# edenartlab/sd-lora-trainer

Measured on AMD Instinct MI355X. Metric: training images/sec, SDXL 1024px rank-16 LoRA, 1/2/4/8 GPU (job-parallel), higher is better.
Workload: dtype bf16

## Files before the change

include/sdlt_kernels.h:

```cpp
#ifndef SDLT_KERNELS_H
#define SDLT_KERNELS_H
#include <stdint.h>
#ifdef __cplusplus
extern "C" {
#endif

const char* sdlt_last_error(void);
int sdlt_abi_version(void);
int sdlt_struct_size(int which);

typedef struct sdlt_gemm_batch_item {
  const void* X; const void* W;
  const void* Adown; const void* Bup; void* T_out;
  void* C; void* Ct;
  const float* bias;
  const float* col_scale;
} sdlt_gemm_batch_item;

typedef struct sdlt_gemm_params {
  const void* X; int64_t ldx;
  const void* W; int64_t ldw;
  int32_t M, N, K;
  const void* X2; int64_t ldx2;
  const void* W2; int64_t ldw2;
// ... 16 lines not shown
  void* Ct; int64_t ldct;
  int32_t splitk;
  int32_t ws_cnt_len;
  void* ws_slab; int64_t ws_slab_bytes;
  int32_t stages;
  int32_t accumulate;
  int32_t* ws_cnt;
  int32_t lora_group_n;
  int32_t lora_group_k;
  const sdlt_gemm_batch_item* batch;
  int32_t n_batch;
  int32_t throughput_hint;
  int32_t epi_op; int32_t epi_act;
  void* epi_out; int64_t ld_epi_out;
  const void* epi_in; int64_t ld_epi_in;
  const float* col_scale;
  const float* ln_c1;
  float* ln_stats;
  const float* ln_adapter;
  float ln_eps;
  int32_t ln_nparts;
  const void* ln_parts;
  int32_t x2_group_n;
} sdlt_gemm_params;
int sdlt_gemm_bf16(const sdlt_gemm_params* p, void* stream);


typedef struct sdlt_lora_grad_desc {
  const void* P; int64_t ldp;
  const void* Q; int64_t ldq;
  float* out;
  int32_t M, Cw, R, Rp;
  int32_t rank_major;
  int32_t accumulate;
  int32_t conv, Hin, Win, Cin, Hout, Wout, stride;
  const void* zero;
  int32_t first_block;
  int32_t pad_;
} sdlt_lora_grad_desc;
int sdlt_lora_grad_grouped(const sdlt_lora_grad_desc* descs_dev, const int32_t* block_desc_dev,
                           int32_t n_blocks, int32_t Rp, int32_t mfma, void* stream);
int32_t sdlt_lora_grad_block_cols(void);
int sdlt_lora_grad_wide(const sdlt_lora_grad_desc* descs_dev, const int32_t* block_desc_dev,
                        int32_t n_blocks, int32_t Rp, int32_t mfma, void* stream);

typedef struct sdlt_attn_params {
// ... 417 lines not shown
```

sd-lora-trainer_amd/_lib.py:

```python
import ctypes as C
import os

import torch

_HERE = os.path.dirname(os.path.abspath(__file__))
LIB_PATH = os.environ.get("SDLT_KERNEL_LIB") or os.path.join(_HERE, "libsdlt_kernels.so")

i32, i64, f32, vp = C.c_int32, C.c_int64, C.c_float, C.c_void_p


class GemmParams(C.Structure):
    _fields_ = [
        ("X", vp), ("ldx", i64), ("W", vp), ("ldw", i64),
        ("M", i32), ("N", i32), ("K", i32),
        ("X2", vp), ("ldx2", i64), ("W2", vp), ("ldw2", i64),
        ("K2", i32), ("mode", i32),
        ("Hin", i32), ("Win", i32), ("Cin", i32), ("Hout", i32), ("Wout", i32),
        ("stride", i32), ("ups", i32), ("flip", i32), ("tr", i32),
        ("zero", vp),
        ("Adown", vp), ("ld_adown", i64), ("Bup", vp), ("ld_bup", i64),
        ("T_out", vp), ("ld_t", i64),
        ("lora_R", i32), ("lora_scale", f32), ("alpha", f32),
        ("bias", vp),
        ("rowbias", vp), ("ld_rowbias", i64), ("rows_per_batch", i32),
        ("R", vp), ("ldr", i64),
        ("C", vp), ("ldc", i64),
        ("out_fp32", i32), ("tile", i32),
        ("Ct", vp), ("ldct", i64),
        ("splitk", i32), ("ws_cnt_len", i32), ("ws_slab", vp), ("ws_slab_bytes", i64), ("stages", i32), ("accumulate", i32), ("ws_cnt", vp),
        ("lora_group_n", i32), ("lora_group_k", i32),
        ("batch", vp), ("n_batch", i32), ("throughput_hint", i32),
        ("epi_op", i32), ("epi_act", i32), ("epi_out", vp), ("ld_epi_out", i64), ("epi_in", vp), ("ld_epi_in", i64),
        ("col_scale", vp),
        ("ln_c1", vp), ("ln_stats", vp), ("ln_adapter", vp), ("ln_eps", f32), ("ln_nparts", i32), ("ln_parts", vp),
        ("x2_group_n", i32),
    ]


class LnFoldDesc(C.Structure):
    _fields_ = [("A32", vp), ("lda", i64), ("gamma", vp), ("beta", vp), ("Ag", vp), ("ldag", i64), ("consts", vp), ("rank", i32), ("K", i32)]


class GemmBatchItem(C.Structure):
    _fields_ = [("X", vp), ("W", vp), ("Adown", vp), ("Bup", vp), ("T_out", vp), ("C", vp), ("Ct", vp), ("bias", vp), ("col_scale", vp)]


class SplitsumDesc(C.Structure):
    _fields_ = [("s0", vp), ("s1", vp), ("ld32", i64), ("out0", vp), ("ldo0", i64), ("out1", vp), ("ldo1", i64),
                ("nsplit", i32), ("B", i32), ("Nk", i32), ("Nkp", i32), ("C", i32), ("acc0", i32), ("nblocks", i32), ("pad_", i32)]


class DoraDesc(C.Structure):
    _fields_ = [("W", vp), ("ldw", i64), ("A", vp), ("lda", i64), ("B", vp), ("ldb", i64), ("mag", vp), ("scale", vp), ("Bt", vp), ("ldbt", i64),
                ("B32", vp), ("ldb32", i64), ("N", i32), ("K", i32), ("Rp", i32), ("rank", i32), ("s", f32), ("pad_", i32)]


class DoraWtDesc(C.Structure):
    _fields_ = [("src", vp), ("dst", vp), ("ld", i64), ("scale", vp), ("rows", i32), ("cols", i32), ("period", i32), ("nvalid", i32)]
# ... 264 lines not shown
```

sd-lora-trainer_amd/csrc/gemm.hip:

```cpp
#include <type_traits>
#include "common.h"
#include "../../include/sdlt_kernels.h"

namespace {

constexpr int BK = 64;
constexpr int ROW_BYTES = 128;

struct ConvGeom {
  int Hin, Win, Cin, Hout, Wout, stride, ups, flip, tr;
};

template <int N_>
__device__ __forceinline__ void wait_vmcnt() { asm volatile("s_waitcnt vmcnt(%0)" ::"n"(N_) : "memory"); }

#ifdef SDLT_GEMM_TRACE
__device__ long long g_gemm_tr[16];
#define GTR(i_) do { if (blockIdx.x == 0 && blockIdx.y == 0 && threadIdx.x == 0) g_gemm_tr[i_] = clock64(); } while (0)
#else
#define GTR(i_) do {} while (0)
#endif

template <int MI, int NI, int WN, int MODE, int R16, int NSTAGE, int KG = 0, int BT = 0, int WM = 2, int EPI = 0, int LN = 0>
__global__ __launch_bounds__(64 * WM * WN) void gemm_kernel(const sdlt_gemm_params p) {
  static_assert(!LN || (MODE == 0 && KG == 0 && BT == 0 && R16 <= 1), "folded LayerNorm: plain products, rank pad 16 at most");
  GTR(0);
  const sdlt_gemm_batch_item* bi = BT ? p.batch + blockIdx.y : nullptr;
  const void* pX = (bi && bi->X) ? bi->X : p.X;
  const void* pW = (bi && bi->W) ? bi->W : p.W;
  const void* pAdown = (bi && bi->Adown) ? bi->Adown : p.Adown;
  const void* pBup = (bi && bi->Bup) ? bi->Bup : p.Bup;
  void* pTout = (bi && bi->T_out) ? bi->T_out : p.T_out;
  void* pC = (bi && bi->C) ? bi->C : p.C;
  void* pCt = (bi && bi->Ct) ? bi->Ct : p.Ct;
  const float* pBias = (bi && bi->bias) ? bi->bias : p.bias;
  const float* pCs = R16 ? ((bi && bi->col_scale) ? bi->col_scale : p.col_scale) : nullptr;
  constexpr int NW = WM * WN, NTHR = NW * 64;
  constexpr int BM = WM * MI * 16, BN = WN * NI * 16;
  static_assert(WM == 2 || WM == 4, "wave rows");
  constexpr int XT = BM * ROW_BYTES, WT = BN * ROW_BYTES, AT = (R16 ? R16 * 16 : 0) * ROW_BYTES;
  constexpr int STAGE = XT + WT + AT;
  constexpr int S = NSTAGE;
  constexpr int TW = (KG ? KG * R16 : R16) * 16;
  constexpr int TROW = R16 ? (TW + 4) : 4;
  static_assert(KG == 0 || R16 >= 1, "K-grouped adapters need an adapter");
  extern __shared__ __attribute__((aligned(16))) char smem[];
  char* tsh = smem + (S == 1 ? 2 : S) * STAGE;
  float* lnsh = (float*)(tsh + (R16 ? BM * TROW * 2 : 0));
// ... 244 lines not shown
      lnca = *(const f32x4*)(p.ln_adapter + lgrp * 32 + fk * 4);
      lnab = *(const f32x4*)(p.ln_adapter + lgrp * 32 + 16 + fk * 4);
    }
  }
  f32x4 lnp[LN == 2 ? 8 : 1];
  if constexpr (LN == 2) {
#pragma unroll
    for (int i = 0; i < 8; ++i) {
      const int tr = tid < BM ? tid : 0;
      const int m = m0 + tr < p.M ? m0 + tr : p.M - 1;
      lnp[i] = *(const f32x4*)((const float*)p.ln_parts + ((size_t)m * p.ln_nparts + (2 * i < p.ln_nparts ? 2 * i : 0)) * 2);
    }
  }
  constexpr int CST = BN + 4;
  constexpr int REGION = (S == 1 ? 2 : S) * STAGE;
  constexpr int CROWS = BM * CST * 4 <= REGION ? BM : (BM / 2 * CST * 4 <= REGION ? BM / 2 : BM / 4);
  static_assert(CROWS * CST * 4 <= REGION && CROWS % 16 == 0, "staged epilogue does not fit the staging LDS");
  constexpr int NCH = BN / 8;
  constexpr int QPP = CROWS * NCH / NTHR;
  constexpr int RIT = (BM / CROWS) * QPP;
  constexpr bool RPRE = RIT <= 4 && QPP * NTHR == CROWS * NCH;
  const bool vec_ok = ((p.ldc & 3) == 0) && (p.R == nullptr || (p.ldr & 3) == 0) &&
                      (p.rowbias == nullptr || (p.ld_rowbias & 3) == 0);
  const bool staged = EPI != 0 ||
                      ((long)p.M * p.N >= (1l << 20) && !p.out_fp32 && pCt == nullptr && vec_ok && (p.ldc & 7) == 0 && (p.N & 7) == 0 &&
                       (p.R == nullptr || (p.ldr & 7) == 0) && (((uintptr_t)pC | (uintptr_t)p.R) & 15) == 0);
  uint4 rpre[RPRE ? RIT : 1];
  const bool rpre_on = RPRE && staged && p.R != nullptr && splitk == 1;
  if (rpre_on) {
#pragma unroll
    for (int t = 0; t < RIT; ++t) {
      const int it = tid + (t % QPP) * NTHR, row = it / NCH, ch = it - row * NCH;
      const int m = m0 + (t / QPP) * CROWS + row, n = n0 + ch * 8;
      rpre[t] = *(const uint4*)((const bf16_t*)p.R + (size_t)(m < p.M ? m : p.M - 1) * p.ldr + (n < p.N ? n : 0));
    }
  }

  GTR(14);
  f32x4 acc[NI][MI];
#pragma unroll
  for (int a = 0; a < NI; ++a)
#pragma unroll
    for (int b = 0; b < MI; ++b) acc[a][b] = (f32x4){0.f, 0.f, 0.f, 0.f};
  constexpr int TMI = MI >= WN ? MI / WN : 1;
  const bool t_active = wn * TMI < MI;
  f32x4 tacc[R16 ? R16 : 1][TMI];
#pragma unroll
// ... 408 lines not shown
          o.x = pack2bf(dh[0], dh[1]); o.y = pack2bf(dh[2], dh[3]); o.z = pack2bf(dh[4], dh[5]); o.w = pack2bf(dh[6], dh[7]);
          *(uint4*)dst = o;
          o.x = pack2bf(dgt[0], dgt[1]); o.y = pack2bf(dgt[2], dgt[3]); o.z = pack2bf(dgt[4], dgt[5]); o.w = pack2bf(dgt[6], dgt[7]);
          *(uint4*)(dst + 16) = o;
          continue;
        }
        if constexpr (EPI == 4) {
          const uint4 pv = *(const uint4*)((const bf16_t*)p.epi_in + (size_t)m * p.ld_epi_in + n);
          const uint32_t* pp = (const uint32_t*)&pv;
          float v8[8] = {lo[0], lo[1], lo[2], lo[3], hi[0], hi[1], hi[2], hi[3]};
#pragma unroll
          for (int j = 0; j < 8; ++j) {
            const float x = bf2f((pp[j >> 1] >> ((j & 1) * 16)) & 0xffff);
            float d;
            if (p.epi_act == 1) { const float sg = 1.f / (1.f + __expf(-1.702f * x)); d = sg + 1.702f * x * sg * (1.f - sg); }
            else d = dgelu_f(x);
            v8[j] *= d;
          }
          lo = (f32x4){v8[0], v8[1], v8[2], v8[3]};
          hi = (f32x4){v8[4], v8[5], v8[6], v8[7]};
        }
        o.x = pack2bf(lo[0], lo[1]); o.y = pack2bf(lo[2], lo[3]); o.z = pack2bf(hi[0], hi[1]); o.w = pack2bf(hi[2], hi[3]);
        *(uint4*)((bf16_t*)pC + (size_t)m * p.ldc + n) = o;
        if constexpr (EPI == 3) {
          float v8[8] = {lo[0], lo[1], lo[2], lo[3], hi[0], hi[1], hi[2], hi[3]};
#pragma unroll
          for (int j = 0; j < 8; ++j) v8[j] = p.epi_act == 1 ? v8[j] / (1.f + __expf(-1.702f * v8[j])) : gelu_f(v8[j]);
          uint4 q;
          q.x = pack2bf(v8[0], v8[1]); q.y = pack2bf(v8[2], v8[3]); q.z = pack2bf(v8[4], v8[5]); q.w = pack2bf(v8[6], v8[7]);
          *(uint4*)((bf16_t*)p.epi_out + (size_t)m * p.ld_epi_out + n) = q;
        }
        if (EPI == 1 && ((n >> 4) & 1) == 0) {
          const f32x4 glo = *(const f32x4*)(src + 16), ghi = *(const f32x4*)(src + 20);
          uint4 q;
          q.x = pack2bf(lo[0] * gelu_f(glo[0]), lo[1] * gelu_f(glo[1])); q.y = pack2bf(lo[2] * gelu_f(glo[2]), lo[3] * gelu_f(glo[3]));
          q.z = pack2bf(hi[0] * gelu_f(ghi[0]), hi[1] * gelu_f(ghi[1])); q.w = pack2bf(hi[2] * gelu_f(ghi[2]), hi[3] * gelu_f(ghi[3]));
          *(uint4*)((bf16_t*)p.epi_out + (size_t)m * p.ld_epi_out + (n >> 5) * 16 + (n & 15)) = q;
        }
      }
      if (pass + 1 < BM / CROWS) __syncthreads();
    }
    GTR(11);
    return;
  }
#endif
#pragma unroll
// ... 38 lines not shown
          *(float4*)((float*)pC + (size_t)m * p.ldc + n) = make_float4(v[0], v[1], v[2], v[3]);
        } else {
          uint2 o;
          o.x = pack2bf(v[0], v[1]); o.y = pack2bf(v[2], v[3]);
          *(uint2*)((bf16_t*)pC + (size_t)m * p.ldc + n) = o;
        }
      } else {
#pragma unroll
        for (int r = 0; r < 4; ++r) {
          if (n + r >= p.N) break;
          float x = v[r] + (pBias ? biasf[a][r] : 0.f);
          if (p.rowbias) x += bf2f(((const bf16_t*)p.rowbias)[(size_t)brow * p.ld_rowbias + n + r]);
          if (p.R) x += bf2f(((const bf16_t*)p.R)[(size_t)m * p.ldr + n + r]);
          if (pCt) ((bf16_t*)pCt)[(size_t)(n + r) * p.ldct + m] = f2bf(x);
          if (p.out_fp32) ((float*)pC)[(size_t)m * p.ldc + n + r] = p.accumulate ? ((float*)pC)[(size_t)m * p.ldc + n + r] + x : x;
          else ((bf16_t*)pC)[(size_t)m * p.ldc + n + r] = f2bf(x);
        }
      }
    }
  }
  GTR(11);
}

template <int MI, int NI, int WN, int MODE, int R16, int NSREQ, int KG = 0, int BT = 0, int WM = 2, int EPI = 0, int LN = 0>
int launch(const sdlt_gemm_params& p, hipStream_t stream) {
  constexpr int NTHR = 64 * WM * WN;
  constexpr int BM = WM * MI * 16, BN = WN * NI * 16;
  constexpr int STAGE = (BM + BN + R16 * 16) * ROW_BYTES;
  constexpr int TSH = (R16 ? BM * ((KG ? KG * R16 : R16) * 16 + 4) * 2 : 0) + (LN ? BM * 8 : 0);
  constexpr int NS = NSREQ <= 2 ? NSREQ : ((4 * STAGE + TSH <= 160 * 1024) ? 4 : ((3 * STAGE + TSH <= 160 * 1024) ? 3 : 2));
  constexpr int NBUF = NS == 1 ? 2 : NS;
  if constexpr (NBUF * STAGE + TSH > 160 * 1024) {
    SDLT_FAIL(SDLT_ERR_UNSUPPORTED, "sdlt_gemm_bf16: tile %dx%d with LoRA rank pad %d does not fit the 160 KB LDS", BM, BN, R16 * 16);
  } else {
  const int smem = NBUF * STAGE + TSH;
  if (sdlt_raise_smem((const void*)gemm_kernel<MI, NI, WN, MODE, R16, NS, KG, BT, WM, EPI, LN>, smem))
    SDLT_FAIL(SDLT_ERR_LAUNCH, "sdlt_gemm_bf16: cannot raise the dynamic LDS limit to %d bytes", smem);
  const int nbm = (p.M + BM - 1) / BM, nbn = (p.N + BN - 1) / BN;
  const int splitk = p.splitk > 1 ? p.splitk : 1;
  if (splitk > 1) {
    constexpr int TMI = MI >= WN ? MI / WN : 1;
    const size_t slab_bytes = (size_t)(NI * MI + (R16 ? R16 * TMI : 0)) * NTHR * 16;
    if (!p.ws_slab || !p.ws_cnt || (size_t)nbm * nbn * splitk * slab_bytes > (size_t)p.ws_slab_bytes || nbm * nbn > p.ws_cnt_len)
      SDLT_FAIL(SDLT_ERR_SHAPE, "sdlt_gemm_bf16: split-K workspace too small (%d tiles x %d splits x %zu B)", nbm * nbn, splitk, slab_bytes);
  }
  hipLaunchKernelGGL((gemm_kernel<MI, NI, WN, MODE, R16, NS, KG, BT, WM, EPI, LN>), dim3(nbm * nbn * splitk, BT ? p.n_batch : 1), dim3(NTHR), smem, stream, p);
  }
  return SDLT_OK;
}

void tile_dims(int tile, int& bm, int& bn) {
  switch (tile) {
    case 7: bm = 256; bn = 160; break;
    case 8: bm = 128; bn = 160; break;
    case 1: case 5: bm = 128; bn = 128; break;
    case 2: bm = 64; bn = 128; break;
    case 4: bm = 256; bn = 128; break;
    case 6: bm = 256; bn = 256; break;
    default: bm = 64; bn = 64; break;
  }
}

template <int MODE, int R16>
int dispatch_tile(const sdlt_gemm_params& pin, hipStream_t s) {
  sdlt_gemm_params p = pin;
  if (p.lora_group_k > 0) {
    const int G = p.K / p.lora_group_k;
    const long t128 = (long)((p.M + 127) / 128) * ((p.N + 127) / 128);
    p.splitk = (pin.splitk == G || (pin.splitk == 0 && G > 1 && t128 * G <= 320 && p.ws_slab && p.ws_cnt)) ? G : 1;
  }
  if (p.batch) p.splitk = 1;
  if (p.ln_c1) p.splitk = 1;
  const int ktot = p.K + p.K2;
  if (p.tile == 0) {
    const long t128 = (long)((p.M + 127) / 128) * ((p.N + 127) / 128);
    const int nk = ktot / BK;
    const bool ws = p.ws_slab && p.ws_cnt;
    if (R16 <= 1 && !p.batch && !p.lora_group_k && p.N % 160 == 0 && p.M > 128 && !p.throughput_hint) {
      const long t7 = (long)((p.M + 255) / 256) * (p.N / 160), t8 = (long)((p.M + 127) / 128) * (p.N / 160);
      if (MODE == 0 && R16 == 0 && ktot <= 2560) {
        if (t7 >= 256) p.tile = 7;
        else if (t8 >= 224) p.tile = 8;
      } else if (MODE == 0 && R16 == 1 && !p.lora_group_n && ktot <= 640 && t8 >= 224 && t8 <= 320) {
        p.tile = 8;
      } else if (MODE != 0 && (t8 == 256 || t8 == 128 || t8 == 64)) {
        const int sk = (int)(256 / t8);
        if (sk == 1 || (ws && !p.splitk && nk / sk >= 16)) { p.tile = 8; if (sk > 1) p.splitk = sk; }
      }
      if (p.tile && !p.splitk) p.splitk = 1;
    }
    if (p.tile) {}
    else if (p.M <= 64) p.tile = p.N > 64 ? 2 : 3;
    else if (p.N <= 64) p.tile = 3;
    else if (p.M <= 128) {
      p.tile = 3;
// ... 48 lines not shown
    const long tiles = (long)((p.M + bm - 1) / bm) * ((p.N + bn - 1) / bn);
    const int nk = ktot / BK;
    int sk = 1;
    if (p.ws_slab && p.ws_cnt && tiles <= 96) {
      sk = (int)((256 + tiles / 2) / tiles);
      const int min_steps = tiles <= 32 ? 3 : 8;
      if (sk > nk / min_steps) sk = nk / min_steps;
      if (sk > 16) sk = 16;
      if (sk < 1) sk = 1;
    }
    p.splitk = sk;
  }
#define SDLT_TILE_CASES(NSV)                                         \
  switch (p.tile) {                                                  \
    case 1: return launch<4, 2, 4, MODE, R16, NSV>(p, s);            \
    case 2: return launch<2, 2, 4, MODE, R16, NSV>(p, s);            \
    case 3: return launch<2, 2, 2, MODE, R16, NSV>(p, s);            \
    case 4: return launch<8, 2, 4, MODE, R16, NSV>(p, s);            \
    case 5: return launch<4, 4, 2, MODE, R16, NSV>(p, s);            \
    case 6: return launch<8, 4, 4, MODE, R16, NSV>(p, s);            \
    case 7: if constexpr (R16 <= 1) return launch<4, 5, 2, MODE, R16, NSV, 0, 0, 4>(p, s); else break; \
    case 8: if constexpr (R16 <= 1) return launch<2, 5, 2, MODE, R16, NSV, 0, 0, 4>(p, s); else break; \
  }
  if (p.ln_c1) {
    const bool parts = p.ln_parts && p.ln_nparts >= 2 && p.ln_nparts <= 16 && !(p.ln_nparts & 1) && !(((uintptr_t)p.ln_parts) & 15);
    if constexpr (MODE == 0 && R16 == 1) {
      if (p.tile != 1 && p.tile != 2 && p.tile != 3 && p.tile != 8) p.tile = (p.lora_group_n > 0 && (p.lora_group_n % 128)) ? 3 : 1;
      if (parts && p.stages != 2) {
        switch (p.tile) {
          case 1: return launch<4, 2, 4, 0, 1, 4, 0, 0, 2, 0, 2>(p, s);
          case 2: return launch<2, 2, 4, 0, 1, 4, 0, 0, 2, 0, 2>(p, s);
        }
      }
      if (p.stages == 2) {
        switch (p.tile) {
          case 1: return launch<4, 2, 4, 0, 1, 2, 0, 0, 2, 0, 1>(p, s);
          case 2: return launch<2, 2, 4, 0, 1, 2, 0, 0, 2, 0, 1>(p, s);
          case 3: return launch<2, 2, 2, 0, 1, 2, 0, 0, 2, 0, 1>(p, s);
          case 8: return launch<2, 5, 2, 0, 1, 2, 0, 0, 4, 0, 1>(p, s);
        }
      } else {
        switch (p.tile) {
          case 1: return launch<4, 2, 4, 0, 1, 4, 0, 0, 2, 0, 1>(p, s);
          case 2: return launch<2, 2, 4, 0, 1, 4, 0, 0, 2, 0, 1>(p, s);
          case 3: return launch<2, 2, 2, 0, 1, 4, 0, 0, 2, 0, 1>(p, s);
          case 8: return launch<2, 5, 2, 0, 1, 4, 0, 0, 4, 0, 1>(p, s);
        }
      }
    }
    if constexpr (MODE == 0 && R16 == 0) {
      if (p.epi_op == 1) {
        if (p.tile == 4 || p.tile == 5 || p.tile == 6) p.tile = 1;
        if (parts && p.tile == 7) return launch<4, 5, 2, 0, 0, 4, 0, 0, 4, 1, 2>(p, s);
        switch (p.tile) {
          case 1: return launch<4, 2, 4, 0, 0, 4, 0, 0, 2, 1, 1>(p, s);
          case 2: return launch<2, 2, 4, 0, 0, 4, 0, 0, 2, 1, 1>(p, s);
// ... 101 lines not shown
  }
  if (p.epi_op) {
    if (p.epi_op < 1 || p.epi_op > 4) SDLT_FAIL(SDLT_ERR_UNSUPPORTED, "sdlt_gemm_bf16: epi_op %d", p.epi_op);
    if (p.mode != 0 || p.lora_R) SDLT_FAIL(SDLT_ERR_UNSUPPORTED, "sdlt_gemm_bf16: fused epilogues exist for plain GEMMs without LoRA");
    const int nmul = p.epi_op == 1 ? 32 : (p.epi_op == 2 ? 16 : 8);
    if (p.out_fp32 || p.Ct || p.batch || p.rowbias || (p.N % nmul) || (p.epi_op != 4 && (!p.epi_out || (p.ld_epi_out & 7) || ((uintptr_t)p.epi_out & 15))))
      SDLT_FAIL(SDLT_ERR_UNSUPPORTED, "sdlt_gemm_bf16: fused epilogue %d needs a bf16 output, no Ct / batch / row bias, N %% %d == 0, 16-byte aligned rows", p.epi_op, nmul);
    if ((p.epi_op == 3 || p.epi_op == 4) && (!p.C || (p.ldc & 7) || ((uintptr_t)p.C & 15) || (p.R && ((p.ldr & 7) || ((uintptr_t)p.R & 15)))))
      SDLT_FAIL(SDLT_ERR_ALIGN, "sdlt_gemm_bf16: fused activation epilogue: C / R rows must be 16-byte aligned");
    if (p.epi_op == 4 && (!p.epi_in || (p.ld_epi_in & 7) || ((uintptr_t)p.epi_in & 15)))
      SDLT_FAIL(SDLT_ERR_ALIGN, "sdlt_gemm_bf16: fused activation backward: pre-activation rows must be 16-byte aligned");
    if (p.epi_op == 1 && (!p.C || (p.ldc & 7) || ((uintptr_t)p.C & 15) || (p.R && ((p.ldr & 7) || ((uintptr_t)p.R & 15)))))
      SDLT_FAIL(SDLT_ERR_ALIGN, "sdlt_gemm_bf16: fused GEGLU forward: C / R rows must be 16-byte aligned");
    if (p.epi_op == 2 && (!p.epi_in || (p.ld_epi_in & 7) || ((uintptr_t)p.epi_in & 15) || p.R))
      SDLT_FAIL(SDLT_ERR_ALIGN, "sdlt_gemm_bf16: fused GEGLU backward: F1 rows must be 16-byte aligned, no residual");
  }
  if (p.ln_c1) {
    if (p.mode != 0 || p.K2 || p.batch || p.alpha != 1.f || p.col_scale || p.lora_group_k > 0 || p.out_fp32 || (p.lora_R && p.lora_R != 16) ||
        (p.lora_R && !p.ln_adapter) || (p.epi_op != 0 && p.epi_op != 1) || (p.splitk > 1))
      SDLT_FAIL(SDLT_ERR_UNSUPPORTED, "sdlt_gemm_bf16: folded LayerNorm needs mode 0, one K segment, alpha 1, bf16 out, lora_R 0 / 16 (+ ln_adapter), epi_op 0 / 1, no batch / DoRA / split-K");
    if ((((uintptr_t)p.ln_c1) & 15) || (((uintptr_t)p.ln_adapter) & 15) || (((uintptr_t)p.ln_stats) & 7))
      SDLT_FAIL(SDLT_ERR_ALIGN, "sdlt_gemm_bf16: ln_c1 / ln_adapter 16-byte, ln_stats 8-byte aligned");
  }
  if (p.accumulate && !p.out_fp32) SDLT_FAIL(SDLT_ERR_UNSUPPORTED, "sdlt_gemm_bf16: accumulate needs an fp32 output (use R for bf16)");
  int r16 = 0;
  if (p.col_scale && !p.lora_R) SDLT_FAIL(SDLT_ERR_UNSUPPORTED, "sdlt_gemm_bf16: col_scale (DoRA) is an option of adapter launches (lora_R > 0)");
  if (p.col_scale && (((uintptr_t)p.col_scale) & 15)) SDLT_FAIL(SDLT_ERR_ALIGN, "sdlt_gemm_bf16: col_scale must be 16-byte aligned");
  if (p.lora_R) {
    if (p.lora_R != 16 && p.lora_R != 32 && p.lora_R != 64) SDLT_FAIL(SDLT_ERR_UNSUPPORTED, "sdlt_gemm_bf16: padded LoRA rank %d (16/32/64)", p.lora_R);
    if (p.K2) SDLT_FAIL(SDLT_ERR_UNSUPPORTED, "sdlt_gemm_bf16: LoRA + second segment");
    if ((p.ld_adown % 8) || (p.ld_bup % 4) || (p.T_out && (p.ld_t % 4))) SDLT_FAIL(SDLT_ERR_ALIGN, "sdlt_gemm_bf16: LoRA operand alignment");
    r16 = p.lora_R / 16;
    if (p.lora_group_k > 0) {
      if (p.lora_group_n > 0 || p.mode != 0 || (p.lora_group_k % BK) || (p.K % p.lora_group_k) || p.K / p.lora_group_k > 4)
        SDLT_FAIL(SDLT_ERR_UNSUPPORTED, "sdlt_gemm_bf16: lora_group_k=%d needs mode 0, K = G*group_k with G <= 4, group_k %% 64 == 0", p.lora_group_k);
    }
  }
  int rc;
#define DISPATCH(MODE_)                                                 \
  switch (r16) {                                                        \
    case 0: rc = dispatch_tile<MODE_, 0>(p, s); break;                  \
    case 1: rc = dispatch_tile<MODE_, 1>(p, s); break;                  \
    case 2: rc = dispatch_tile<MODE_, 2>(p, s); break;                  \
    default: rc = dispatch_tile<MODE_, 4>(p, s); break;                 \
  }
  if (p.mode == 0) { DISPATCH(0) } else if (p.K2) { rc = dispatch_tile<2, 0>(p, s); } else { DISPATCH(1) }
// ... 6 lines not shown
```

sd-lora-trainer_amd/ops.py:

```python
import ctypes as C
import os
import weakref

import torch

from . import _lib

BF16 = torch.bfloat16
F32 = torch.float32


def _stream():
    return C.c_void_p(torch.cuda.current_stream().cuda_stream)


def _p(t):
    return C.c_void_p(t.data_ptr()) if t is not None else C.c_void_p(0)


def _ld(t):
    assert t.dim() == 2 and t.stride(1) == 1, f"need a 2-D row-major view, got {tuple(t.shape)} strides {t.stride()}"
    return t.stride(0)


# ... 191 lines not shown
        _PF["mode"] = None
        return None
    _PF["idx"] = i + 1
    if i + 1 < len(seq) and seq[i + 1][0] and seq[i + 1][0] != ent[0] and seq[i + 1][1] % 320 == 0:
        return seq[i + 1]
    return None


WSK_CONV = os.environ.get("SDLT_WSK_CONV", "1") != "0"


def wsk_conv_shape(conv, N, lora_rank_pad=0):
    if not (WSK and WSK_CONV) or conv.stride != 1 or conv.ups != 1 or conv.tr or conv.Hin != conv.Hout or conv.Win != conv.Wout:
        return False
    M = conv.B * conv.Hout * conv.Wout
    if M % 64 or N % 640 or conv.Cin % 64 or lora_rank_pad not in (0, 16):
        return False
    return 200 <= (M // 64) * (N // 80) <= 256


def gemm_emits_parts(M, N, K, lora_rank_pad=0, W=None, dora=False):
    ok = (WSK and not THROUGHPUT_HINT and (WSK_DORA or not dora) and (lora_rank_pad in (0, 16) or (lora_rank_pad in WSK_RANKS and WSK_PACK and W is not None and _wsk_is_frozen(W))) and wsk_shape(M, N, K, lora_rank_pad > 0)
          and (N // 80) % 2 == 0 and N // 80 <= 16)
    return N // 80 if ok else 0


def _wsk_gemm_route(X, W, lora, *, conv, rowbias, col_scale, lora_group_k, ln):
    rp_ = lora[0].shape[0] if lora is not None else 0
    return (WSK and conv is None and rowbias is None and (col_scale is None or (lora is not None and ln is None and WSK_DORA)) and (ln is None or not lora_group_k)
            and (lora is None or (rp_ == 16 and ((not lora_group_k and lora[1].shape[1] == 16) or
                                                 (lora_group_k and lora_group_k % 64 == 0 and W.shape[1] // lora_group_k in (2, 3))))
                 or (rp_ in WSK_RANKS and rp_ > 16 and not lora_group_k and ln is None and lora[1].shape[1] == rp_ and WSK_PACK and _wsk_is_frozen(W)))
            and wsk_shape(X.shape[0], W.shape[0], W.shape[1], lora is not None))


def _wsk_conv_route(W, lora, *, conv, col_scale, lora_group_k, ln):
    return (conv is not None and col_scale is None and not lora_group_k and ln is None and (lora is None or (lora[0].shape[0] == 16 and lora[1].shape[1] == 16))
            and wsk_conv_shape(conv, W.shape[0], 16 if lora is not None else 0))


def _gemm_wsk(X, W, out, *, lora, bias, residual, lora_group_k, col_scale, ln, ln_parts_out, rowdot, out0):
    _chk2(X), _chk2(W), _chk2(out)
    M_, N_, K_ = X.shape[0], W.shape[0], W.shape[1]
    assert X.shape[1] == K_ and tuple(out.shape) == (M_, N_)
    q = _lib.WskGemmParams()
    Wptr, Wld = _wsk_operand(W)
    q.X, q.ldx, q.W, q.ldw, q.M, q.N, q.K = _p(X), _ld(X), Wptr, Wld, M_, N_, K_
# ... 51 lines not shown
    A_ = B_ = T_ = None
    scale_ = 0.0
    if lora is not None:
        A_, B_, scale_, T_ = lora
        _chk2(A_), _chk2(B_)
        assert tuple(A_.shape) == (16, 9 * conv.Cin) and tuple(B_.shape) == (N_, 16) and (T_ is None or tuple(T_.shape) == (M_, 16))
    if bias is not None:
        _chk2(bias, F32)
    if rowbias is not None:
        _chk2(rowbias)
        assert rowbias.shape[1] == N_ and rows_per_batch == conv.Hout * conv.Wout and rowbias.shape[0] >= conv.B
    if residual is not None:
        _chk2(residual)
        assert tuple(residual.shape) == (M_, N_)
    Wptr, Wld = _wsk_operand(W)
    _lib.check(_lib.load().sdlt_wsk_conv(_p(X), _ld(X), Wptr, Wld, conv.B, conv.Hout, conv.Wout, conv.Cin, N_, int(conv.flip), _p(bias), _p(rowbias),
                                         _ld(rowbias) if rowbias is not None else 0, _p(residual), _ld(residual) if residual is not None else 0, _p(out), _ld(out),
                                         _p(A_), _ld(A_) if A_ is not None else 0, _p(B_), _ld(B_) if B_ is not None else 0, float(scale_), _p(T_),
                                         _ld(T_) if T_ is not None else 0, _p(zero_page(X.device)), _stream()), "sdlt_wsk_conv")
    return out


def _gemm_tiled(X, W, out, *, X2, W2, conv, lora, bias, rowbias, rows_per_batch, residual, alpha, Ct, tile, splitk, stages, accumulate, lora_group_n, lora_group_k, batch,
                geglu_out, geglu_bwd, act_out, dact_in, col_scale, ln, x2_group_n):
    lib = _lib.load()
    p = _lib.GemmParams()
    _chk2(X), _chk2(W)
    p.X, p.ldx, p.W, p.ldw = _p(X), _ld(X), _p(W), _ld(W)
    N, K = W.shape
    if conv is None:
        M = X.shape[0]
        assert X.shape[1] == K, (X.shape, W.shape)
        p.mode = 0
    else:
        M = conv.B * conv.Hout * conv.Wout
        assert K == 9 * conv.Cin and X.shape[1] == conv.Cin and X.shape[0] == conv.B * conv.Hin * conv.Win
        p.mode = 1
        p.Hin, p.Win, p.Cin, p.Hout, p.Wout = conv.Hin, conv.Win, conv.Cin, conv.Hout, conv.Wout
        p.stride, p.ups, p.flip, p.tr = conv.stride, conv.ups, conv.flip, conv.tr
        p.zero = _p(zero_page(X.device))
    p.M, p.N, p.K = M, N, K
    p.throughput_hint = int(THROUGHPUT_HINT)
    if X2 is not None:
        _chk2(X2), _chk2(W2)
        G2 = 1
        if x2_group_n:
            assert conv is None and batch is None and N % x2_group_n == 0
# ... 57 lines not shown
        p.epi_act = int(kind == "quick_gelu")
        if act_out is not None:
            p.epi_op, p.epi_out, p.ld_epi_out = 3, _p(t), _ld(t)
        else:
            p.epi_op, p.epi_in, p.ld_epi_in = 4, _p(t), _ld(t)
    if geglu_out is not None:
        _chk2(geglu_out)
        assert tuple(geglu_out.shape) == (M, N // 2) and geglu_bwd is None
        p.epi_op, p.epi_out, p.ld_epi_out = 1, _p(geglu_out), _ld(geglu_out)
    if Ct is not None:
        _chk2(Ct)
        assert Ct.shape[0] == N and Ct.shape[1] >= M
        p.Ct, p.ldct = _p(Ct), _ld(Ct)
    p.tile, p.splitk, p.stages, p.accumulate = tile, splitk, stages, int(accumulate)
    if ln is not None:
        c1, stats_, eps_, lnad = ln[:4]
        _chk2(c1, F32)
        assert c1.numel() == N and (stats_ is None or (stats_.dtype == F32 and stats_.numel() >= 2 * M)) and (lora is None or lnad is not None)
        p.ln_c1, p.ln_stats, p.ln_eps, p.ln_adapter = _p(c1), _p(stats_), float(eps_), _p(lnad)
        if len(ln) > 4 and ln[4] is not None:
            parts, npart = ln[4], int(ln[5])
            assert parts.dtype == F32 and parts.is_contiguous() and parts.numel() >= M * npart * 2
            p.ln_parts, p.ln_nparts = _p(parts), npart
    if batch is not None:
        p.batch, p.n_batch = _p(batch.dev), batch.n
    slab, cnt = splitk_workspace(X.device)
    p.ws_slab, p.ws_slab_bytes, p.ws_cnt, p.ws_cnt_len = _p(slab), slab.numel(), _p(cnt), cnt.numel()
    _lib.check(lib.sdlt_gemm_bf16(C.byref(p), _stream()), "sdlt_gemm_bf16")
    return out if geglu_bwd is None else geglu_bwd[1]


def gemm(X, W, out, *, X2=None, W2=None, conv=None, lora=None, bias=None, rowbias=None, rows_per_batch=0,
         residual=None, alpha=1.0, Ct=None, tile=0, splitk=0, stages=0, accumulate=False, lora_group_n=0, lora_group_k=0, batch=None,
         geglu_out=None, geglu_bwd=None, act_out=None, dact_in=None, col_scale=None, ln=None, ln_parts_out=None, rowdot=None, out0=None,
         x2_group_n=0):
    assert lora is None or (lora[0].shape[0] if lora_group_k else lora[1].shape[1]) <= 64, "fused adapter products exist for rank pads 16 / 32 / 64"
    assert X2 is None or lora is None, "a second K segment excludes the fused adapter"
    if out0 is not None:
        assert residual is not None and lora is not None and Ct is None and ln is None and geglu_out is None and act_out is None and tuple(out0.shape) == tuple(out.shape)
    plain = (X2 is None and alpha == 1.0 and Ct is None and batch is None and geglu_out is None and geglu_bwd is None and act_out is None and dact_in is None and not accumulate
             and tile == 0 and splitk == 0 and not lora_group_n and out is not None and out.dtype == BF16 and not THROUGHPUT_HINT)
    if plain and _wsk_gemm_route(X, W, lora, conv=conv, rowbias=rowbias, col_scale=col_scale, lora_group_k=lora_group_k, ln=ln):
        return _gemm_wsk(X, W, out, lora=lora, bias=bias, residual=residual, lora_group_k=lora_group_k, col_scale=col_scale, ln=ln, ln_parts_out=ln_parts_out, rowdot=rowdot, out0=out0)
    assert ln_parts_out is None, "ln_parts_out: this product does not run on the wave-split-K kernel (ops.gemm_emits_parts)"
    if out0 is not None:
        gemm(X, W, out0, lora=lora, bias=bias, col_scale=col_scale, tile=tile, splitk=splitk, stages=stages, lora_group_n=lora_group_n, lora_group_k=lora_group_k)
        return add2d(out0, residual, out)
    if plain and _wsk_conv_route(W, lora, conv=conv, col_scale=col_scale, lora_group_k=lora_group_k, ln=ln):
        return _gemm_wsk_conv(X, W, out, conv=conv, lora=lora, bias=bias, rowbias=rowbias, rows_per_batch=rows_per_batch, residual=residual)
    return _gemm_tiled(X, W, out, X2=X2, W2=W2, conv=conv, lora=lora, bias=bias, rowbias=rowbias, rows_per_batch=rows_per_batch, residual=residual, alpha=alpha, Ct=Ct, tile=tile,
                       splitk=splitk, stages=stages, accumulate=accumulate, lora_group_n=lora_group_n, lora_group_k=lora_group_k, batch=batch, geglu_out=geglu_out,
                       geglu_bwd=geglu_bwd, act_out=act_out, dact_in=dact_in, col_scale=col_scale, ln=ln, x2_group_n=x2_group_n)


STRIP_SPLITK = int(os.environ.get("SDLT_STRIP_SPLITK", "1"))


def strip_splitk(N, K, B):
    s = max(1, STRIP_SPLITK)
    return s if (K // 256) >= s else 1


def strip_partial_splits(N, K, B):
    strips = N // 16
    s = max(1, min(8, 256 // max(1, strips * B), (K // 256) // 3))
    return s


STRIP_WIDE_MIN = int(os.environ.get("SDLT_STRIP_WIDE_MIN", "2304"))


class _PairQueue:
    def __init__(self):
        self.pending = []
        self.launches = 0
# ... 1136 lines not shown
```

sd-lora-trainer_amd/unet.py:

```python
import copy
import os
import math

import torch

from . import ops as _ops
from .topology import CONFIGS, TIME_DIM_MULT, lora_targets, param_shapes

BF16, F32 = torch.bfloat16, torch.float32


def _pad_to(x, m):
    return (x + m - 1) // m * m


XATTN_WGS = int(os.environ.get("SDLT_XATTN_WGS", "160"))

LORA_WIDE_MIN = int(os.environ.get("SDLT_LORA_WIDE_MIN", "128"))
LORA_MAX_RANK = 256


def padded_rank(rank):
    if rank <= 64:
        return 16 if rank <= 16 else (32 if rank <= 32 else 64)
# ... 1015 lines not shown

    def backward(self, dx3, dctx):
        rt = self.rt
        if self.fused_geglu:
            f1 = self.ff1._b["y"]
            df1 = rt.ops.gemm(dx3, self.ff2.Wt, None, geglu_bwd=(f1, self.buf("df1", *f1.shape)))
        else:
            dg = self.ff2.backward(dx3)
            df1 = rt.ops.geglu_bwd(self.ff1._b["y"], dg, self.buf("df1", *self.ff1._b["y"].shape))
        dx2 = self.norm3.backward(self.ff1.backward(df1), dres=dx3)
        dx1 = self.norm2.backward(self.attn2.backward(dx2, dctx), dres=dx2)
        return self.norm1.backward(self.attn1.backward(dx1), dres=dx1)


class Transformer2D(_Module):
    def __init__(self, rt, name, sd, arena, C, heads, nlayers, hooked):
        super().__init__(rt, name)
        self.norm = GroupNorm(rt, name + ".norm", sd, 1e-6, silu=False)
        self.proj_in = Linear(rt, name + ".proj_in", sd)
        self.blocks = [TransformerBlock(rt, f"{name}.transformer_blocks.{k}", sd, arena, heads, hooked) for k in range(nlayers)]
        self.proj_out = Linear(rt, name + ".proj_out", sd)

    def forward(self, x, ctx, B, HW):
        h = self.proj_in.forward(self.norm.forward(x, None, B, HW))
        self.blocks[0].norm1._parts = None
        for i, blk in enumerate(self.blocks):
            h = blk.forward(h, ctx, B, HW, next_norm=self.blocks[i + 1].norm1 if i + 1 < len(self.blocks) else None)
        return self.proj_out.forward(h, residual=x)

    def backward(self, dout, dctx):
        dh = self.proj_out.backward(dout)
        for blk in reversed(self.blocks):
            dh = blk.backward(dh, dctx)
        return self.norm.backward(self.proj_in.backward(dh), dres=dout)


class ResnetBlock(_Module):
    def __init__(self, rt, name, sd, arena, cin1, cin2, cout):
        super().__init__(rt, name)
        self.cin1, self.cin2, self.cout = cin1, cin2, cout
        self.norm1 = GroupNorm(rt, name + ".norm1", sd, 1e-5, silu=True)
        self.conv1 = Conv3x3(rt, name + ".conv1", sd)
        self.temb = Linear(rt, name + ".time_emb_proj", sd)
        self.norm2 = GroupNorm(rt, name + ".norm2", sd, 1e-5, silu=True)
        self.conv2 = Conv3x3(rt, name + ".conv2", sd, arena)
        self.shortcut = None
        if (name + ".conv_shortcut.weight") in sd:
            self.shortcut = Linear(rt, name + ".conv_shortcut", sd)
# ... 433 lines not shown
```

Measured before the change: 24.65.

## Emit LayerNorm row partials from tiled GEMM epilogue for N=640 products

Adds a SIDE variant of the tiled GEMM that, in its staged epilogue, reduces each output row's bf16 values over 32/64/128-column groups with DPP cross-lane sums and writes per-group sum and centred sum-of-squares. The next LayerNorm can then use these precomputed partials (folded-LN parts path) instead of a separate statistics pass, which now also covers products that do not route to the wave-split-K kernel, such as Transformer proj_in. A new 2-stage parts-enabled folded-LN launch is added too. In exchange the GEMM is pinned to one tile shape with 4 stages and no split-K, and its epilogue does extra reduction work.

```diff
diff --git a/include/sdlt_kernels.h b/include/sdlt_kernels.h
--- a/include/sdlt_kernels.h
+++ b/include/sdlt_kernels.h
@@ -62,6 +62,8 @@
   int32_t ln_nparts;
   const void* ln_parts;
   int32_t x2_group_n;
+  int32_t ln_parts_w;
+  void* ln_parts_out;
 } sdlt_gemm_params;
 int sdlt_gemm_bf16(const sdlt_gemm_params* p, void* stream);
 
diff --git a/sd-lora-trainer_amd/_lib.py b/sd-lora-trainer_amd/_lib.py
--- a/sd-lora-trainer_amd/_lib.py
+++ b/sd-lora-trainer_amd/_lib.py
@@ -33,7 +33,7 @@
         ("epi_op", i32), ("epi_act", i32), ("epi_out", vp), ("ld_epi_out", i64), ("epi_in", vp), ("ld_epi_in", i64),
         ("col_scale", vp),
         ("ln_c1", vp), ("ln_stats", vp), ("ln_adapter", vp), ("ln_eps", f32), ("ln_nparts", i32), ("ln_parts", vp),
-        ("x2_group_n", i32),
+        ("x2_group_n", i32), ("ln_parts_w", i32), ("ln_parts_out", vp),
     ]
 
 
diff --git a/sd-lora-trainer_amd/csrc/gemm.hip b/sd-lora-trainer_amd/csrc/gemm.hip
--- a/sd-lora-trainer_amd/csrc/gemm.hip
+++ b/sd-lora-trainer_amd/csrc/gemm.hip
@@ -13,6 +13,18 @@
 
 template <int N_>
 __device__ __forceinline__ void wait_vmcnt() { asm volatile("s_waitcnt vmcnt(%0)" ::"n"(N_) : "memory"); }
+
+template <int CTRL>
+__device__ __forceinline__ float dpp_move(float v) {
+  return __builtin_bit_cast(float, __builtin_amdgcn_update_dpp(0, __builtin_bit_cast(int, v), CTRL, 0xf, 0xf, false));
+}
+__device__ __forceinline__ float group_allsum(float v, int lanes) {
+  v += dpp_move<0xB1>(v);
+  v += dpp_move<0x4E>(v);
+  if (lanes > 4) v += dpp_move<0x141>(v);
+  if (lanes > 8) v += dpp_move<0x140>(v);
+  return v;
+}
 
 #ifdef SDLT_GEMM_TRACE
 __device__ long long g_gemm_tr[16];
@@ -21,9 +33,10 @@
 #define GTR(i_) do {} while (0)
 #endif
 
-template <int MI, int NI, int WN, int MODE, int R16, int NSTAGE, int KG = 0, int BT = 0, int WM = 2, int EPI = 0, int LN = 0>
+template <int MI, int NI, int WN, int MODE, int R16, int NSTAGE, int KG = 0, int BT = 0, int WM = 2, int EPI = 0, int LN = 0, int SIDE = 0>
 __global__ __launch_bounds__(64 * WM * WN) void gemm_kernel(const sdlt_gemm_params p) {
   static_assert(!LN || (MODE == 0 && KG == 0 && BT == 0 && R16 <= 1), "folded LayerNorm: plain products, rank pad 16 at most");
+  static_assert(!SIDE || (MODE == 0 && KG == 0 && BT == 0 && R16 <= 1 && EPI == 0 && LN == 0), "row partials: plain products, rank pad 16 at most");
   GTR(0);
   const sdlt_gemm_batch_item* bi = BT ? p.batch + blockIdx.y : nullptr;
   const void* pX = (bi && bi->X) ? bi->X : p.X;
@@ -314,7 +327,7 @@
   constexpr bool RPRE = RIT <= 4 && QPP * NTHR == CROWS * NCH;
   const bool vec_ok = ((p.ldc & 3) == 0) && (p.R == nullptr || (p.ldr & 3) == 0) &&
                       (p.rowbias == nullptr || (p.ld_rowbias & 3) == 0);
-  const bool staged = EPI != 0 ||
+  const bool staged = EPI != 0 || SIDE != 0 ||
                       ((long)p.M * p.N >= (1l << 20) && !p.out_fp32 && pCt == nullptr && vec_ok && (p.ldc & 7) == 0 && (p.N & 7) == 0 &&
                        (p.R == nullptr || (p.ldr & 7) == 0) && (((uintptr_t)pC | (uintptr_t)p.R) & 15) == 0);
   uint4 rpre[RPRE ? RIT : 1];
@@ -769,6 +782,19 @@
         }
         o.x = pack2bf(lo[0], lo[1]); o.y = pack2bf(lo[2], lo[3]); o.z = pack2bf(hi[0], hi[1]); o.w = pack2bf(hi[2], hi[3]);
         *(uint4*)((bf16_t*)pC + (size_t)m * p.ldc + n) = o;
+        if constexpr (SIDE == 1) {
+          static_assert(NCH == 16 && (NTHR % 16) == 0, "row partials: 128-column tiles");
+          const float y8[8] = {bf2f(o.x & 0xffff), bf2f(o.x >> 16), bf2f(o.y & 0xffff), bf2f(o.y >> 16), bf2f(o.z & 0xffff), bf2f(o.z >> 16), bf2f(o.w & 0xffff), bf2f(o.w >> 16)};
+          const int gl = p.ln_parts_w >> 3, gsh = 31 - __builtin_clz(p.ln_parts_w);
+          const float sx = group_allsum(((y8[0] + y8[1]) + (y8[2] + y8[3])) + ((y8[4] + y8[5]) + (y8[6] + y8[7])), gl);
+          const float mg = sx / (float)p.ln_parts_w;
+          float m2 = 0.f;
+#pragma unroll
+          for (int j = 0; j < 8; ++j) m2 += (y8[j] - mg) * (y8[j] - mg);
+          m2 = group_allsum(m2, gl);
+          if ((ch & (gl - 1)) == 0)
+            *(float2*)((float*)p.ln_parts_out + ((size_t)m * (p.N >> gsh) + (n >> gsh)) * 2) = make_float2(sx, m2);
+        }
         if constexpr (EPI == 3) {
           float v8[8] = {lo[0], lo[1], lo[2], lo[3], hi[0], hi[1], hi[2], hi[3]};
 #pragma unroll
@@ -853,7 +879,7 @@
   GTR(11);
 }
 
-template <int MI, int NI, int WN, int MODE, int R16, int NSREQ, int KG = 0, int BT = 0, int WM = 2, int EPI = 0, int LN = 0>
+template <int MI, int NI, int WN, int MODE, int R16, int NSREQ, int KG = 0, int BT = 0, int WM = 2, int EPI = 0, int LN = 0, int SIDE = 0>
 int launch(const sdlt_gemm_params& p, hipStream_t stream) {
   constexpr int NTHR = 64 * WM * WN;
   constexpr int BM = WM * MI * 16, BN = WN * NI * 16;
@@ -865,7 +891,7 @@
     SDLT_FAIL(SDLT_ERR_UNSUPPORTED, "sdlt_gemm_bf16: tile %dx%d with LoRA rank pad %d does not fit the 160 KB LDS", BM, BN, R16 * 16);
   } else {
   const int smem = NBUF * STAGE + TSH;
-  if (sdlt_raise_smem((const void*)gemm_kernel<MI, NI, WN, MODE, R16, NS, KG, BT, WM, EPI, LN>, smem))
+  if (sdlt_raise_smem((const void*)gemm_kernel<MI, NI, WN, MODE, R16, NS, KG, BT, WM, EPI, LN, SIDE>, smem))
     SDLT_FAIL(SDLT_ERR_LAUNCH, "sdlt_gemm_bf16: cannot raise the dynamic LDS limit to %d bytes", smem);
   const int nbm = (p.M + BM - 1) / BM, nbn = (p.N + BN - 1) / BN;
   const int splitk = p.splitk > 1 ? p.splitk : 1;
@@ -875,7 +901,7 @@
     if (!p.ws_slab || !p.ws_cnt || (size_t)nbm * nbn * splitk * slab_bytes > (size_t)p.ws_slab_bytes || nbm * nbn > p.ws_cnt_len)
       SDLT_FAIL(SDLT_ERR_SHAPE, "sdlt_gemm_bf16: split-K workspace too small (%d tiles x %d splits x %zu B)", nbm * nbn, splitk, slab_bytes);
   }
-  hipLaunchKernelGGL((gemm_kernel<MI, NI, WN, MODE, R16, NS, KG, BT, WM, EPI, LN>), dim3(nbm * nbn * splitk, BT ? p.n_batch : 1), dim3(NTHR), smem, stream, p);
+  hipLaunchKernelGGL((gemm_kernel<MI, NI, WN, MODE, R16, NS, KG, BT, WM, EPI, LN, SIDE>), dim3(nbm * nbn * splitk, BT ? p.n_batch : 1), dim3(NTHR), smem, stream, p);
   }
   return SDLT_OK;
 }
@@ -902,6 +928,7 @@
   }
   if (p.batch) p.splitk = 1;
   if (p.ln_c1) p.splitk = 1;
+  if (p.ln_parts_out) { p.tile = 1; p.splitk = 1; p.stages = 4; }
   const int ktot = p.K + p.K2;
   if (p.tile == 0) {
     const long t128 = (long)((p.M + 127) / 128) * ((p.N + 127) / 128);
@@ -996,6 +1023,10 @@
     case 7: if constexpr (R16 <= 1) return launch<4, 5, 2, MODE, R16, NSV, 0, 0, 4>(p, s); else break; \
     case 8: if constexpr (R16 <= 1) return launch<2, 5, 2, MODE, R16, NSV, 0, 0, 4>(p, s); else break; \
   }
+  if (p.ln_parts_out) {
+    if constexpr (MODE == 0 && R16 <= 1) return launch<4, 2, 4, 0, R16, 4, 0, 0, 2, 0, 0, 1>(p, s);
+    SDLT_FAIL(SDLT_ERR_UNSUPPORTED, "sdlt_gemm_bf16: ln_parts_out needs mode 0 and lora_R 0 / 16 (lora_R %d)", p.lora_R);
+  }
   if (p.ln_c1) {
     const bool parts = p.ln_parts && p.ln_nparts >= 2 && p.ln_nparts <= 16 && !(p.ln_nparts & 1) && !(((uintptr_t)p.ln_parts) & 15);
     if constexpr (MODE == 0 && R16 == 1) {
@@ -1006,6 +1037,7 @@
           case 2: return launch<2, 2, 4, 0, 1, 4, 0, 0, 2, 0, 2>(p, s);
         }
       }
+      if (parts && p.stages == 2 && p.tile == 1) return launch<4, 2, 4, 0, 1, 2, 0, 0, 2, 0, 2>(p, s);
       if (p.stages == 2) {
         switch (p.tile) {
           case 1: return launch<4, 2, 4, 0, 1, 2, 0, 0, 2, 0, 1>(p, s);
@@ -1153,6 +1185,14 @@
     if ((((uintptr_t)p.ln_c1) & 15) || (((uintptr_t)p.ln_adapter) & 15) || (((uintptr_t)p.ln_stats) & 7))
       SDLT_FAIL(SDLT_ERR_ALIGN, "sdlt_gemm_bf16: ln_c1 / ln_adapter 16-byte, ln_stats 8-byte aligned");
   }
+  if (p.ln_parts_out) {
+    if (p.mode != 0 || p.K2 || p.batch || p.ln_c1 || p.epi_op || p.lora_group_k > 0 || p.lora_group_n > 0 || p.out_fp32 || p.Ct || p.splitk > 1 || (p.lora_R && p.lora_R != 16))
+      SDLT_FAIL(SDLT_ERR_UNSUPPORTED, "sdlt_gemm_bf16: ln_parts_out needs mode 0, one K segment, bf16 out, lora_R 0 / 16, no batch / adapter groups / fused epilogue / Ct / folded LayerNorm / split-K");
+    if ((p.ln_parts_w != 32 && p.ln_parts_w != 64 && p.ln_parts_w != 128) || (p.N % p.ln_parts_w))
+      SDLT_FAIL(SDLT_ERR_SHAPE, "sdlt_gemm_bf16: ln_parts_w=%d must be 32, 64 or 128 and divide N=%d", p.ln_parts_w, p.N);
+    if (!p.C || (p.ldc & 7) || (p.R && (p.ldr & 7)) || (p.rowbias && (p.ld_rowbias & 3)) || (((uintptr_t)p.C | (uintptr_t)p.R) & 15) || (((uintptr_t)p.ln_parts_out) & 7))
+      SDLT_FAIL(SDLT_ERR_ALIGN, "sdlt_gemm_bf16: ln_parts_out: C / R rows must be 16-byte aligned, the partials 8-byte");
+  }
   if (p.accumulate && !p.out_fp32) SDLT_FAIL(SDLT_ERR_UNSUPPORTED, "sdlt_gemm_bf16: accumulate needs an fp32 output (use R for bf16)");
   int r16 = 0;
   if (p.col_scale && !p.lora_R) SDLT_FAIL(SDLT_ERR_UNSUPPORTED, "sdlt_gemm_bf16: col_scale (DoRA) is an option of adapter launches (lora_R > 0)");
diff --git a/sd-lora-trainer_amd/ops.py b/sd-lora-trainer_amd/ops.py
--- a/sd-lora-trainer_amd/ops.py
+++ b/sd-lora-trainer_amd/ops.py
@@ -237,7 +237,33 @@
 def gemm_emits_parts(M, N, K, lora_rank_pad=0, W=None, dora=False):
     ok = (WSK and not THROUGHPUT_HINT and (WSK_DORA or not dora) and (lora_rank_pad in (0, 16) or (lora_rank_pad in WSK_RANKS and WSK_PACK and W is not None and _wsk_is_frozen(W))) and wsk_shape(M, N, K, lora_rank_pad > 0)
           and (N // 80) % 2 == 0 and N // 80 <= 16)
-    return N // 80 if ok else 0
+    if ok:
+        return N // 80
+    return tiled_parts_count(M, N, K, lora_rank_pad, dora)
+
+
+PARTS_TILED = os.environ.get("SDLT_LN_PARTS_TILED", "1") != "0"
+
+
+def tiled_parts_width(N):
+    for w in (128, 64, 32):
+        if N % w == 0 and (N // w) % 2 == 0 and N // w <= 16:
+            return w
+    return 0
+
+
+def tiled_parts_count(M, N, K, lora_rank_pad=0, dora=False):
+    if not PARTS_TILED or THROUGHPUT_HINT or dora or lora_rank_pad not in (0, 16) or N != 640 or M <= 128 or K % 64 or K > 6144:
+        return 0
+    t128 = ((M + 127) // 128) * ((N + 127) // 128)
+    if not 160 <= t128 < 320:
+        return 0
+    if N % 160 == 0:
+        t7, t8 = ((M + 255) // 256) * (N // 160), ((M + 127) // 128) * (N // 160)
+        if (lora_rank_pad == 0 and K <= 2560 and (t7 >= 256 or t8 >= 224)) or (lora_rank_pad == 16 and K <= 640 and 224 <= t8 <= 320):
+            return 0
+    w = tiled_parts_width(N)
+    return N // w if w else 0
 
 
 def _wsk_gemm_route(X, W, lora, *, conv, rowbias, col_scale, lora_group_k, ln):
@@ -335,7 +361,7 @@
 
 
 def _gemm_tiled(X, W, out, *, X2, W2, conv, lora, bias, rowbias, rows_per_batch, residual, alpha, Ct, tile, splitk, stages, accumulate, lora_group_n, lora_group_k, batch,
-                geglu_out, geglu_bwd, act_out, dact_in, col_scale, ln, x2_group_n):
+                geglu_out, geglu_bwd, act_out, dact_in, col_scale, ln, x2_group_n, ln_parts_out=None):
     lib = _lib.load()
     p = _lib.GemmParams()
     _chk2(X), _chk2(W)
@@ -439,6 +465,10 @@
             parts, npart = ln[4], int(ln[5])
             assert parts.dtype == F32 and parts.is_contiguous() and parts.numel() >= M * npart * 2
             p.ln_parts, p.ln_nparts = _p(parts), npart
+    if ln_parts_out is not None:
+        w = tiled_parts_width(N)
+        assert w and ln is None and conv is None and ln_parts_out.dtype == F32 and ln_parts_out.is_contiguous() and ln_parts_out.numel() >= M * (N // w) * 2
+        p.ln_parts_out, p.ln_parts_w = _p(ln_parts_out), w
     if batch is not None:
         p.batch, p.n_batch = _p(batch.dev), batch.n
     slab, cnt = splitk_workspace(X.device)
@@ -459,7 +489,7 @@
              and tile == 0 and splitk == 0 and not lora_group_n and out is not None and out.dtype == BF16 and not THROUGHPUT_HINT)
     if plain and _wsk_gemm_route(X, W, lora, conv=conv, rowbias=rowbias, col_scale=col_scale, lora_group_k=lora_group_k, ln=ln):
         return _gemm_wsk(X, W, out, lora=lora, bias=bias, residual=residual, lora_group_k=lora_group_k, col_scale=col_scale, ln=ln, ln_parts_out=ln_parts_out, rowdot=rowdot, out0=out0)
-    assert ln_parts_out is None, "ln_parts_out: this product does not run on the wave-split-K kernel (ops.gemm_emits_parts)"
+    assert ln_parts_out is None or (plain and col_scale is None and out0 is None and not lora_group_k and conv is None), "ln_parts_out: a plain or rank-16-adapter product"
     if out0 is not None:
         gemm(X, W, out0, lora=lora, bias=bias, col_scale=col_scale, tile=tile, splitk=splitk, stages=stages, lora_group_n=lora_group_n, lora_group_k=lora_group_k)
         return add2d(out0, residual, out)
@@ -467,7 +497,7 @@
         return _gemm_wsk_conv(X, W, out, conv=conv, lora=lora, bias=bias, rowbias=rowbias, rows_per_batch=rows_per_batch, residual=residual)
     return _gemm_tiled(X, W, out, X2=X2, W2=W2, conv=conv, lora=lora, bias=bias, rowbias=rowbias, rows_per_batch=rows_per_batch, residual=residual, alpha=alpha, Ct=Ct, tile=tile,
                        splitk=splitk, stages=stages, accumulate=accumulate, lora_group_n=lora_group_n, lora_group_k=lora_group_k, batch=batch, geglu_out=geglu_out,
-                       geglu_bwd=geglu_bwd, act_out=act_out, dact_in=dact_in, col_scale=col_scale, ln=ln, x2_group_n=x2_group_n)
+                       geglu_bwd=geglu_bwd, act_out=act_out, dact_in=dact_in, col_scale=col_scale, ln=ln, x2_group_n=x2_group_n, ln_parts_out=ln_parts_out)
 
 
 STRIP_SPLITK = int(os.environ.get("SDLT_STRIP_SPLITK", "1"))
diff --git a/sd-lora-trainer_amd/unet.py b/sd-lora-trainer_amd/unet.py
--- a/sd-lora-trainer_amd/unet.py
+++ b/sd-lora-trainer_amd/unet.py
@@ -1061,8 +1061,7 @@
         self.proj_out = Linear(rt, name + ".proj_out", sd)
 
     def forward(self, x, ctx, B, HW):
-        h = self.proj_in.forward(self.norm.forward(x, None, B, HW))
-        self.blocks[0].norm1._parts = None
+        h = self.proj_in.forward(self.norm.forward(x, None, B, HW), parts_for=self.blocks[0].norm1)
         for i, blk in enumerate(self.blocks):
             h = blk.forward(h, ctx, B, HW, next_norm=self.blocks[i + 1].norm1 if i + 1 < len(self.blocks) else None)
         return self.proj_out.forward(h, residual=x)
```

New measurement: 24.64. About the same (-0.1%).
